# mwaurawakati/hotstuff-digital-signature-benchmarking

Measured on AMD Instinct MI355X. Metric: Ed25519 verifies/sec at batch 2^20 per GPU (bit-exact ed25519-dalek verify_strict flags), higher is better.
Workload: dtype u32; 1 GPU; C4: 2^20 independent (pk, 32-B digest, sig) triples per GPU, inputs resident in HBM; batch_per_gpu=1048576, global_batch=1048576, parallelism=dp1 (contiguous shards, no collective on the data path), kernel_variant=21, streams=3

## Files before the change

### hotstuff-digital-signature-benchmarking_amd/csrc/hsv_kernels.hip

```cpp
#include <hip/hip_runtime.h>

#include <algorithm>
#include <cstdlib>
#include <cstring>
#include <type_traits>
#include <atomic>
#include <mutex>
#include <unordered_map>

#include "hsv_internal.h"
#include "hsv_verify_core.hpp"
#include "hsv_verify_hc.hpp"
#include "hsv_rowpoint.hpp"
#include "hsv_pointpass.hpp"
#include "hsv_msgwave.hpp"

namespace hsv {

#ifdef HSV_PHASE_CLOCKS
constexpr uint32_t kPhaseCap = 1u << 16;
__device__ uint64_t g_phase_clk[kPhaseCap * 8];
#endif

template <int WA>
__global__ void __launch_bounds__(kBlock)
hsv_prep_kernel(const uint8_t *__restrict__ pk, uint64_t pk_stride, const uint8_t *__restrict__ sig,
                uint64_t sig_stride, const uint8_t *__restrict__ msg, uint64_t msg_stride, uint32_t n,
                uint32_t *__restrict__ rec, HcCounters *__restrict__ ctr, uint32_t *__restrict__ fb_list,
                int lat_bits) {
  __builtin_amdgcn_s_setprio(3);
  const uint32_t idx = blockIdx.x * kBlock + threadIdx.x;
  if (idx >= n) return;
  uint32_t pkw[8], sigw[16], msgw[8];
  load_triple(pk, pk_stride, sig, sig_stride, msg, msg_stride, idx, pkw, sigw, msgw);
  if (prep_scalars<WA>(pkw, sigw, msgw, rec + idx, n, lat_bits)) fb_list[atomicAdd(&ctr->fb_count, 1u)] = idx;
}

template <int WA, int WAVES, int CB, bool KREC = false>
__global__ void __launch_bounds__(kBlock, WAVES)
hsv_verify_hp_kernel(const uint8_t *__restrict__ pk, uint64_t pk_stride, const uint8_t *__restrict__ sig,
                     uint64_t sig_stride, const uint8_t *__restrict__ msg, uint64_t msg_stride, uint32_t n,
                     uint8_t *__restrict__ flags_out, uint32_t *__restrict__ strict_bits,
                     uint4 *__restrict__ vt_ws, const uint32_t *__restrict__ comb_b,
                     const uint32_t *__restrict__ rec, HcCounters *__restrict__ ctr,
                     const uint32_t *__restrict__ fb_list, uint32_t *__restrict__ canary, uint32_t nonce,
                     uint32_t inject, uint32_t *__restrict__ fault) {
  constexpr int kEnt = (1 << (WA - 1)) + 1;
  const uint32_t slot = blockIdx.x * kBlock + threadIdx.x;
  GlobalVarTab<kEnt> vt{vt_ws + (uint64_t)slot * vt_lane_uint4<WA>(), inject};
  const uint32_t lane = threadIdx.x & 63u;
  canary[slot] = nonce;
  uint32_t bad = 0;
  const uint32_t nfb = __builtin_amdgcn_readfirstlane(ctr->fb_count);
  const uint32_t fb_end = (nfb + 63u) & ~63u;
  const uint32_t words = (n + 31u) / 32u;
#ifdef HSV_PHASE_CLOCKS
  uint32_t nbw = 0;
#endif
  for (;;) {
    uint32_t base = 0;
    if (lane == 0) base = atomicAdd(&ctr->next, 64u);
    base = __builtin_amdgcn_readfirstlane(__shfl(base, 0));
    if (base >= fb_end + n) break;
    if (inject == kInjectCanary) canary[slot] = ~nonce;
    if (base < fb_end) {
      const uint32_t j = base + lane;
      const bool valid = j < nfb;
      const uint32_t idx = fb_list[valid ? j : base];
      uint32_t pkw[8], sigw[16];
      uint32_t f;
      if constexpr (KREC) {
        const uint4 *p = reinterpret_cast<const uint4 *>(pk + (uint64_t)idx * pk_stride);
        const uint4 *s = reinterpret_cast<const uint4 *>(sig + (uint64_t)idx * sig_stride);
        HSV_UNROLL
        for (int j = 0; j < 2; ++j) {
          const uint4 v = p[j];
          pkw[4 * j] = v.x; pkw[4 * j + 1] = v.y; pkw[4 * j + 2] = v.z; pkw[4 * j + 3] = v.w;
        }
        HSV_UNROLL
        for (int j = 0; j < 4; ++j) {
          const uint4 v = s[j];
          sigw[4 * j] = v.x; sigw[4 * j + 1] = v.y; sigw[4 * j + 2] = v.z; sigw[4 * j + 3] = v.w;
        }
        sc k;
        HSV_UNROLL
        for (int i = 0; i < 8; ++i) k.v[i] = rec[(10ull + (uint64_t)i) * n + idx];
        f = verify_one_full_comb<WA, false, CB>(pkw, sigw, k, comb_b, vt);
      } else {
        uint32_t msgw[8];
        load_triple(pk, pk_stride, sig, sig_stride, msg, msg_stride, idx, pkw, sigw, msgw);
        f = verify_one_full_comb<WA, false, CB>(pkw, sigw, msgw, comb_b, vt);
      }
      bad |= ((f & kFault) ? 1u : 0u) | (canary[slot] != nonce ? 2u : 0u);
      if (valid) {
        if (flags_out) flags_out[idx] = (uint8_t)f;
        if (strict_bits && (f & kStrictOk)) atomicOr(&strict_bits[idx >> 5], 1u << (idx & 31u));
      }
      continue;
    }
    const uint32_t b0 = base - fb_end;
    const uint32_t idx = b0 + lane;
    const bool valid = idx < n;
    const uint32_t li = valid ? idx : n - 1u;
    uint32_t pkw[8], rw[8];
    {
      const uint4 *p = reinterpret_cast<const uint4 *>(pk + (uint64_t)li * pk_stride);
      const uint4 *r = reinterpret_cast<const uint4 *>(sig + (uint64_t)li * sig_stride);
      const uint4 p0 = p[0], p1 = p[1], r0 = r[0], r1 = r[1];
      pkw[0] = p0.x; pkw[1] = p0.y; pkw[2] = p0.z; pkw[3] = p0.w;
      pkw[4] = p1.x; pkw[5] = p1.y; pkw[6] = p1.z; pkw[7] = p1.w;
      rw[0] = r0.x; rw[1] = r0.y; rw[2] = r0.z; rw[3] = r0.w;
      rw[4] = r1.x; rw[5] = r1.y; rw[6] = r1.z; rw[7] = r1.w;
    }
    const uint32_t meta = rec[18ull * n + li];
    const bool own = valid && !(meta & kPrepFallback);
#ifdef HSV_PHASE_CLOCKS
    uint64_t clk[5];
    ++nbw;
    const uint64_t cyc0 = clock64();
    clk[0] = wall_clock64();
    const uint32_t f = verify_one_prepped<WA, CB>(pkw, rw, rec + li, n, meta, comb_b, vt, clk);
    clk[4] = wall_clock64();
    {
      uint64_t v = 1;
      HSV_UNROLL
      for (int j = 0; j < 5; ++j) v = lane == (uint32_t)j ? clk[j] : v;
      v = lane == 5u ? (uint64_t)__builtin_amdgcn_s_getreg((31 << 11) | (0 << 6) | 4) : v;
      v = lane == 6u ? ((uint64_t)blockIdx.x << 8 | nbw) : v;
      v = lane == 7u ? (0x100u | (uint64_t)__builtin_amdgcn_s_getreg((3 << 11) | (0 << 6) | 20) |
                        ((clock64() - cyc0) << 16))
                     : v;
      if (lane < 8u && b0 / 64u < kPhaseCap) g_phase_clk[(uint64_t)(b0 / 64u) * 8u + lane] = v;
    }
#else
    const uint32_t f = verify_one_prepped<WA, CB>(pkw, rw, rec + li, n, meta, comb_b, vt);
#endif
    bad |= ((f & kFault) ? 1u : 0u) | (canary[slot] != nonce ? 2u : 0u);
    const uint32_t fo = KREC && (meta & kPrepVoid) ? 0u : f;
    if (own && flags_out) flags_out[idx] = (uint8_t)fo;
    if (strict_bits) {
      const uint64_t mask = __ballot(own && (fo & kStrictOk));
      const uint32_t w = b0 / 32u + lane;
      const uint32_t part = lane ? (uint32_t)(mask >> 32) : (uint32_t)mask;
      if (lane < 2u && w < words && part) atomicOr(&strict_bits[w], part);
    }
  }
  report_faults(fault, bad);
}



template <int CB>
__device__ __forceinline__ ge_ext comb_add_b_half(ge_ext q, const uint32_t s[8], const uint32_t *tb, uint32_t h) {
  constexpr int NP = 256 / CB, HALF = NP / 2;
  constexpr int ENT = 1 << (CB - 1);
  uint32_t sr[9];
  recode_add<9, CB, NP>(s, 8, sr);
  HSV_UNROLL
  for (int i = 0; i < 4; ++i) sr[i] = h ? sr[i + 4] : sr[i];
  HSV_NOUNROLL
  for (int j = 0; j < HALF; ++j) {
    const uint32_t cb = sr[0] & ((1u << CB) - 1u);
    HSV_UNROLL
    for (int i = 0; i < 3; ++i) sr[i] = (sr[i] >> CB) | (sr[i + 1] << (32 - CB));
    sr[3] >>= CB;
    const CombPosTab tpb{tb + (uint64_t)(j + (int)h * HALF) * ENT * kCombEntryWords};
    q = ge_add_niels<true>(q, select_niels<CB>(tpb, cb));
  }
  return q;
}

__device__ __forceinline__ fe fe_swap_pair(const fe &a) {
  fe r;
  HSV_UNROLL
  for (int i = 0; i < kFeLimbs; ++i) r.v[i] = (uint32_t)__shfl_xor((int)a.v[i], 1, 64);
  return r;
}

template <int WA, class VT>
__device__ __forceinline__ void pair_point_phase(uint32_t p, const uint32_t pk[8], const uint32_t rb[8], VT &vt,
                                                 uint32_t &ok, uint32_t &small) {
  constexpr int TS = 1 << (WA - 1);
  uint32_t pt[8];
  HSV_UNROLL
  for (int i = 0; i < 8; ++i) pt[i] = p ? pk[i] : rb[i];
  fe x, y;
  ok = ge_decompress(pt, x, y);
  small = ok & y_is_small_order(y);
// ... 702 lines not shown

uint32_t next_nonce() {
  static std::atomic<uint32_t> ctr{0x9e3779b9u};
  return (ctr.fetch_add(0x61c88646u) * 2654435761u) | 1u;
}


struct TxPrep {
  const uint8_t *txs;
  const uint64_t *offsets;
  uint64_t tx_size;
  uint8_t *records;
};
struct MsgPrep {
  const uint8_t *msgs;
  const uint64_t *offsets;
  uint64_t msg_len, msg_stride;
};

template <int WA, int WAVES, int CB>
hipError_t launch_hp(const uint8_t *pk, uint64_t pk_stride, const uint8_t *sig, uint64_t sig_stride,
                     const uint8_t *msg, uint64_t msg_stride, uint32_t n, uint8_t *flags_out,
                     uint32_t *strict_bits, const uint32_t *comb_b, uint32_t *fault, hipStream_t stream,
                     const TxPrep *tx = nullptr, void *ws_in = nullptr, size_t ws_cap = 0,
                     size_t *ws_need = nullptr, const MsgPrep *mp = nullptr) {
  const void *kern = mp ? reinterpret_cast<const void *>(hsv::hsv_verify_hp_kernel<WA, WAVES, CB, true>)
                        : reinterpret_cast<const void *>(hsv::hsv_verify_hp_kernel<WA, WAVES, CB>);
  int dev = 0;
  hipError_t e = hipGetDevice(&dev);
  if (e != hipSuccess) return e;
  static std::mutex mu;
  static std::unordered_map<int, std::pair<int, int>> slots_per_dev;
  int bpc = 1, cus = 1;
  {
    std::lock_guard<std::mutex> lk(mu);
    auto it = slots_per_dev.find(2 * dev + (mp ? 1 : 0));
    if (it == slots_per_dev.end()) {
      int b = 0, c = 0;
      e = hipOccupancyMaxActiveBlocksPerMultiprocessor(&b, kern, hsv::kBlock, 0);
      if (e != hipSuccess) return e;
      e = hipDeviceGetAttribute(&c, hipDeviceAttributeMultiprocessorCount, dev);
      if (e != hipSuccess) return e;
      it = slots_per_dev.emplace(2 * dev + (mp ? 1 : 0), std::make_pair(std::max(1, b), std::max(1, c))).first;
    }
    bpc = it->second.first;
    cus = it->second.second;
  }
  const bool fused = tx && WA == 4 && WAVES == HSV_HP_WAVES && CB == 16 && tx_fused_enabled() &&
                     (uint64_t)n * 128u <= 0xffffffffull && hsv_tx_fused_blocks_per_cu(dev) > 0;
  if (fused) bpc = std::min(bpc, hsv_tx_fused_blocks_per_cu(dev));
  const int resident = bpc * (hsvi_resident_started() && cus > 1 ? cus - 1 : cus);
  const uint32_t blocks_needed = (n + hsv::kBlock - 1) / hsv::kBlock;
  const uint32_t grid = std::min<uint32_t>(blocks_needed, (uint32_t)resident);
  const size_t ws_bytes = (size_t)grid * hsv::kBlock * hsv::vt_lane_uint4<WA>() * sizeof(uint4);
  const size_t canary_bytes = ((size_t)grid * hsv::kBlock * sizeof(uint32_t) + 255) & ~(size_t)255;
  const size_t fb_bytes = (size_t)n * sizeof(uint32_t);
  const size_t rec_bytes = (size_t)n * hsv::kPrepWords * sizeof(uint32_t);
  const size_t ready_bytes = fused ? (((size_t)(n + 63u) / 64u) * sizeof(uint32_t) + 255) & ~(size_t)255 : 0;
  const size_t need = ws_bytes + 256 + canary_bytes + fb_bytes + rec_bytes + ready_bytes;
  if (ws_need) {
    *ws_need = need;
    return hipSuccess;
  }
  hsv::Workspace ws(ws_in, ws_cap, need, stream);
  if (ws.status() != hipSuccess) return ws.status();
  uint8_t *ws8 = ws.get();
  uint4 *vt_ws = reinterpret_cast<uint4 *>(ws8);
  hsv::HcCounters *ctr = reinterpret_cast<hsv::HcCounters *>(ws8 + ws_bytes);
  uint32_t *canary = reinterpret_cast<uint32_t *>(ws8 + ws_bytes + 256);
  uint32_t *fb_list = reinterpret_cast<uint32_t *>(ws8 + ws_bytes + 256 + canary_bytes);
  uint32_t *rec = reinterpret_cast<uint32_t *>(ws8 + ws_bytes + 256 + canary_bytes + fb_bytes);
  uint32_t *ready = reinterpret_cast<uint32_t *>(ws8 + ws_bytes + 256 + canary_bytes + fb_bytes + rec_bytes);
  e = hipMemsetAsync(ctr, 0, sizeof(hsv::HcCounters), stream);
  if (e == hipSuccess && strict_bits) e = hipMemsetAsync(strict_bits, 0, (size_t)((n + 31u) / 32u) * 4u, stream);
  if (e == hipSuccess && fused) {
    e = hipMemsetAsync(ready, 0, ready_bytes, stream);
    if (e == hipSuccess)
      e = hsv_launch_tx_fused(grid, tx->txs, tx->offsets, tx->tx_size, n, tx->records, rec, ctr, fb_list, ready,
                              g_lat_bits.load(), flags_out, strict_bits, vt_ws, comb_b, canary, next_nonce(), t_inject,
                              fault, stream);
    return ws.done(e);
  }
  if (e == hipSuccess && tx) {
    static_assert(WA == 4, "hsv_launch_tx_prep writes the WA = 4 prepass record");
    e = hsv_launch_tx_prep(tx->txs, tx->offsets, tx->tx_size, n, tx->records, rec, &ctr->fb_count, fb_list,
                           g_lat_bits.load(), stream);
    pk = tx->records;
    sig = tx->records + 32;
    msg = tx->records + 96;
    pk_stride = sig_stride = msg_stride = 128;
  } else if (e == hipSuccess && mp) {
    static_assert(WA == 4, "hsv_launch_msg_prep writes the WA = 4 prepass record");
    e = hsv_launch_msg_prep(pk, pk_stride, sig, sig_stride, mp->msgs, mp->offsets, mp->msg_len, mp->msg_stride, n,
                            rec, &ctr->fb_count, fb_list, g_lat_bits.load(), stream);
  } else if (e == hipSuccess) {
    hipLaunchKernelGGL((hsv::hsv_prep_kernel<WA>), dim3(blocks_needed), dim3(hsv::kBlock), 0, stream, pk, pk_stride,
                       sig, sig_stride, msg, msg_stride, n, rec, ctr, fb_list, g_lat_bits.load());
    e = hipGetLastError();
  }
  if (e == hipSuccess) {
    if (mp) {
      hipLaunchKernelGGL((hsv::hsv_verify_hp_kernel<WA, WAVES, CB, true>), dim3(grid), dim3(hsv::kBlock), 0, stream,
                         pk, pk_stride, sig, sig_stride, nullptr, 0, n, flags_out, strict_bits, vt_ws, comb_b, rec,
                         ctr, fb_list, canary, next_nonce(), t_inject, fault);
    } else {
      hipLaunchKernelGGL((hsv::hsv_verify_hp_kernel<WA, WAVES, CB>), dim3(grid), dim3(hsv::kBlock), 0, stream, pk,
                         pk_stride, sig, sig_stride, msg, msg_stride, n, flags_out, strict_bits, vt_ws, comb_b, rec,
                         ctr, fb_list, canary, next_nonce(), t_inject, fault);
    }
    e = hipGetLastError();
  }
  return ws.done(e);
}

constexpr uint32_t kPairMax = 1u << 13;
constexpr uint32_t kRowMaxDefault = 3072;

constexpr uint32_t row_max() { return kRowMaxDefault; }

constexpr uint32_t kMsgQuadMax = hsv::kQuadMax;
constexpr uint32_t kMsgJointMax = hsv::kJointMax;
constexpr uint32_t kMsgRowMax = kRowMaxDefault;
enum SmallFormId : int { kFormQuad = 1, kFormJoint = 2, kFormRow = 3, kFormPair = 4 };

template <int WA, int CB, bool MSG = false>
struct SmallForm {
  decltype(&hsv::hsv_verify_quad_kernel<WA, CB, MSG>) kern;
  uint32_t grid, block;
  size_t slots;
  int id;
  explicit SmallForm(uint32_t n, int force = 0) {
    id = force                                        ? force
         : n <= (MSG ? kMsgQuadMax : hsv::kQuadMax)   ? kFormQuad
         : n <= (MSG ? kMsgJointMax : hsv::kJointMax) ? kFormJoint
         : n <= (MSG ? kMsgRowMax : row_max())        ? kFormRow
                                                      : kFormPair;
    if (id == kFormQuad) {
      kern = hsv::hsv_verify_quad_kernel<WA, CB, MSG>;
      grid = n, block = 4 * 64, slots = (size_t)grid * 2u;
    } else if (id == kFormJoint) {
      kern = hsv::hsv_verify_joint_kernel<WA, CB, MSG>;
      grid = (n + hsv::kJointItems - 1) / hsv::kJointItems, block = (hsv::kJointItems + 1) * 64;
      slots = (size_t)grid * hsv::kJointItems;
    } else if (id == kFormRow) {
      kern = hsv::hsv_verify_row_kernel<WA, CB, 1, MSG>;
// ... 238 lines not shown
```

### hotstuff-digital-signature-benchmarking_amd/csrc/hsv_mempool.hip

```cpp
#include <hip/hip_runtime.h>

#include <algorithm>
#include <mutex>
#include <unordered_map>

#define HSV_SHA_BITOP3 1
#include "hsv_internal.h"
#include "hsv_keytab.hpp"
#include "hsv_stage.hpp"
#include "hsv_txhash.hpp"
#include "hsv_verify_hc.hpp"
#include "hsv_pointpass.hpp"
#include "hsv_routed.hpp"

namespace hsv {

constexpr int kTxBlock = 256;

__device__ __forceinline__ bool tx_span(const uint64_t *offsets, uint64_t tx_size, uint32_t i, uint64_t &lo,
                                        uint64_t &hi) {
  if (offsets) {
    lo = offsets[i];
    hi = offsets[i + 1];
  } else {
// ... 40 lines not shown
  const uint64_t q_last = ok ? (start + (hi - lo) - 1) >> 4 : kNoChunk;
  uint64_t h[8];
  sha512_init(h);
  const uint64_t nblocks = tx_num_blocks(mlen);
  uint32_t wave_blocks = (uint32_t)nblocks;
  HSV_UNROLL
  for (int m = 1; m < 64; m <<= 1) wave_blocks = max(wave_blocks, (uint32_t)__shfl_xor((int)wave_blocks, m, 64));
  const uint32_t sh16 = (uint32_t)(start & 15u);
  const bool wave_aligned = __all(sh16 == 0u);
  HSV_NOUNROLL
  for (uint32_t b = 0; b < wave_blocks; ++b) {
    uint32_t raw[4 * kTxQ + 1];
    tx_stage_chunks<kTxQ>(q, stage, lane, (start >> 4) + 8ull * b, q_last, raw);
    const bool wave_full = __all((uint64_t)(b + 1u) * 128u <= mlen);
    if (b < nblocks) {
      uint32_t words[32];
      if (wave_aligned) {
        HSV_UNROLL
        for (int j = 0; j < 32; ++j) words[j] = raw[j];
      } else {
        tx_realign<32>(raw, sh16, words);
      }
      if (wave_full) tx_compress_full_block(h, words);
      else tx_compress_block(h, words, mlen, b, nblocks);
    }
  }
  {
    const uint64_t tail = start + mlen;
    uint32_t raw[4 * 7 + 1];
    tx_stage_chunks<7>(q, stage, lane, tail >> 4, q_last, raw);
    tx_realign<24>(raw, (uint32_t)(tail & 15u), r);
  }
  tx_digest_words(h, r + 24);
  if (!ok) {
    HSV_UNROLL
    for (int j = 0; j < 32; ++j) r[j] = 0u;
  }
  return ok;
}

template <bool PREP, bool CLAMP, class Rec, class Put>
__device__ __forceinline__ void tx_record_lane(const uint8_t *__restrict__ txs, const uint64_t *__restrict__ offsets,
                                               uint64_t tx_size, uint32_t n, uint32_t i_in, uint32_t lane,
                                               uint4 *stage, const Rec &out, uint32_t *__restrict__ prep,
                                               uint32_t *__restrict__ fb_count, uint32_t *__restrict__ fb_list,
                                               int lat_bits) {
  const uint32_t i = CLAMP && i_in >= n ? n - 1u : i_in;
  uint32_t r[32];
  (void)tx_record_words(txs, offsets, tx_size, n, i, lane, stage, r);
  if (CLAMP || i < n) {
    HSV_UNROLL
    for (int j = 0; j < 8; ++j) out.put(i, j, r);
    if constexpr (PREP) {
      const bool fallback = prep_scalars<4, Put>(r, r + 8, r + 24, prep + i, n, lat_bits);
      if (fallback && i == i_in) Put::u32(fb_list + atomicAdd(fb_count, 1u), i);
    }
  }
}

template <bool PREP>
__global__ void __launch_bounds__(kTxBlock) hsv_tx_record_kernel(const uint8_t *__restrict__ txs,
                                                                  const uint64_t *__restrict__ offsets,
                                                                  uint64_t tx_size, uint32_t n,
                                                                  uint4 *__restrict__ rec,
                                                                  uint32_t *__restrict__ prep,
                                                                  uint32_t *__restrict__ fb_count,
                                                                  uint32_t *__restrict__ fb_list, int lat_bits) {
  __shared__ uint4 stage_all[kTxWaves][64 * kTxQ];
  if constexpr (PREP) __builtin_amdgcn_s_setprio(3);
  const uint32_t lane = threadIdx.x & 63u, wv = threadIdx.x >> 6;
  if (blockIdx.x * kTxBlock + wv * 64u >= n) return;
  tx_record_lane<PREP, false, TxRecPlain, PutPlain>(txs, offsets, tx_size, n, blockIdx.x * kTxBlock + threadIdx.x, lane,
                                             stage_all[wv], TxRecPlain{rec}, prep, fb_count, fb_list, lat_bits);
}

constexpr uint64_t kTxFusedWaitTicks = 50000000ull;

__device__ __forceinline__ bool tx_wait_word(uint32_t *w, uint32_t want) {
  const uint64_t t0 = wall_clock64();
  for (;;) {
    const uint32_t v = __builtin_amdgcn_readfirstlane(__hip_atomic_load((gu32 *)w, __ATOMIC_RELAXED, __HIP_MEMORY_SCOPE_AGENT));
    if (v >= want) return true;
    if (wall_clock64() - t0 > kTxFusedWaitTicks) return false;
    __builtin_amdgcn_s_sleep(8);
  }
}

template <int WA, int WAVES, int CB>
__global__ void __launch_bounds__(kBlock, WAVES)
hsv_verify_tx_fused_kernel(const uint8_t *__restrict__ txs, const uint64_t *__restrict__ offsets, uint64_t tx_size,
                           uint32_t n, uint8_t *__restrict__ records,
                           uint32_t *__restrict__ rec, HcCounters *__restrict__ ctr, uint32_t *__restrict__ fb_list,
                           uint32_t *__restrict__ ready, int lat_bits, uint8_t *__restrict__ flags_out,
                           uint32_t *__restrict__ strict_bits, uint4 *__restrict__ vt_ws,
                           const uint32_t *__restrict__ comb_b, uint32_t *__restrict__ canary, uint32_t nonce,
                           uint32_t inject, uint32_t *__restrict__ fault) {
  static_assert(kBlock == kTxBlock, "one staging slot per wave");
  __shared__ uint4 stage_all[kBlock / 64][64 * kTxQ];
  constexpr int kEnt = (1 << (WA - 1)) + 1;
  const uint32_t slot = blockIdx.x * kBlock + threadIdx.x;
  GlobalVarTab<kEnt> vt{vt_ws + (uint64_t)slot * vt_lane_uint4<WA>(), inject};
  const uint32_t lane = threadIdx.x & 63u;
  uint4 *stage = stage_all[threadIdx.x >> 6];
  canary[slot] = nonce;
  uint32_t bad = 0;
  const uint32_t nbatch = (n + 63u) / 64u;
  const __amdgpu_buffer_rsrc_t rec_rsrc = __builtin_amdgcn_make_buffer_rsrc(records, 0, (int)(n * 128u), 0x00020000);
  __builtin_amdgcn_s_setprio(3);
  for (;;) {
    uint32_t rb = 0;
    if (lane == 0) rb = atomicAdd(&ctr->rnext, 1u);
    rb = __builtin_amdgcn_readfirstlane(__shfl(rb, 0));
    if (rb >= nbatch) break;
    tx_record_lane<true, true, TxRecWriteThrough, PutWriteThrough>(txs, offsets, tx_size, n, rb * 64u + lane, lane, stage,
                                                             TxRecWriteThrough{rec_rsrc}, rec, &ctr->fb_count,
                                                             fb_list, lat_bits);
    asm volatile("s_waitcnt vmcnt(0)" ::: "memory");
    if (lane < 2u && !(inject == kInjectNoPublish && rb == 0u))
      __hip_atomic_fetch_add((gu32 *)(lane ? &ctr->rdone : ready + rb), 1u, __ATOMIC_RELAXED, __HIP_MEMORY_SCOPE_AGENT);
  }
  __builtin_amdgcn_s_setprio(0);
  const uint32_t words = (n + 31u) / 32u;
  for (;;) {
    uint32_t base = 0;
    if (lane == 0) base = atomicAdd(&ctr->next, 64u);
    base = __builtin_amdgcn_readfirstlane(__shfl(base, 0));
    if (base >= n) break;
    if (inject == kInjectCanary) canary[slot] = ~nonce;
    if ((bad & 4u) || !tx_wait_word(ready + base / 64u, 1u)) {
      bad |= 5u;
      continue;
    }
    __builtin_amdgcn_fence(__ATOMIC_ACQUIRE, "agent");
    const uint32_t idx = base + lane;
    const bool valid = idx < n;
    const uint32_t li = valid ? idx : n - 1u;
    uint32_t pkw[8], rw[8];
    {
      const uint4 *p = reinterpret_cast<const uint4 *>(records + (uint64_t)li * 128u);
      const uint4 p0 = p[0], p1 = p[1], r0 = p[2], r1 = p[3];
      pkw[0] = p0.x; pkw[1] = p0.y; pkw[2] = p0.z; pkw[3] = p0.w;
      pkw[4] = p1.x; pkw[5] = p1.y; pkw[6] = p1.z; pkw[7] = p1.w;
      rw[0] = r0.x; rw[1] = r0.y; rw[2] = r0.z; rw[3] = r0.w;
      rw[4] = r1.x; rw[5] = r1.y; rw[6] = r1.z; rw[7] = r1.w;
    }
    const uint32_t meta = rec[18ull * n + li];
    const bool own = valid && !(meta & kPrepFallback);
    const uint32_t f = verify_one_prepped<WA, CB>(pkw, rw, rec + li, n, meta, comb_b, vt);
    bad |= ((f & kFault) ? 1u : 0u) | (canary[slot] != nonce ? 2u : 0u);
    if (own && flags_out) flags_out[idx] = (uint8_t)f;
    if (strict_bits) {
      const uint64_t mask = __ballot(own && (f & kStrictOk));
      const uint32_t w = base / 32u + lane;
      const uint32_t part = lane ? (uint32_t)(mask >> 32) : (uint32_t)mask;
      if (lane < 2u && w < words && part) atomicOr(&strict_bits[w], part);
    }
  }
  if (!(bad & 4u) && tx_wait_word(&ctr->rdone, nbatch)) {
    __builtin_amdgcn_fence(__ATOMIC_ACQUIRE, "agent");
    const uint32_t nfb =
        __builtin_amdgcn_readfirstlane(__hip_atomic_load((gu32 *)&ctr->fb_count, __ATOMIC_RELAXED, __HIP_MEMORY_SCOPE_AGENT));
    for (;;) {
      uint32_t base = 0;
      if (lane == 0) base = atomicAdd(&ctr->fb_next, 64u);
      base = __builtin_amdgcn_readfirstlane(__shfl(base, 0));
      if (base >= nfb) break;
      const uint32_t j = base + lane;
      const bool valid = j < nfb;
      const uint32_t idx = fb_list[valid ? j : base];
      uint32_t pkw[8], sigw[16], msgw[8];
      load_triple(records, 128, records + 32, 128, records + 96, 128, idx, pkw, sigw, msgw);
      const uint32_t f = verify_one_full_comb<WA, false, CB>(pkw, sigw, msgw, comb_b, vt);
      bad |= ((f & kFault) ? 1u : 0u) | (canary[slot] != nonce ? 2u : 0u);
      if (valid) {
        if (flags_out) flags_out[idx] = (uint8_t)f;
        if (strict_bits && (f & kStrictOk)) atomicOr(&strict_bits[idx >> 5], 1u << (idx & 31u));
      }
    }
  } else {
    bad |= 1u;
  }
  report_faults(fault, bad & 3u);
}

__global__ void __launch_bounds__(kTxBlock) hsv_tx_mask_kernel(const uint64_t *__restrict__ offsets, uint32_t n,
                                                                uint8_t *flags, uint32_t *strict_bits) {
  const uint32_t i = blockIdx.x * kTxBlock + threadIdx.x;
  if (i >= n) return;
  uint64_t lo, hi;
  if (tx_span(offsets, 0, i, lo, hi)) return;
  if (flags) flags[i] = 0;
  if (strict_bits) atomicAnd(strict_bits + (i >> 5), ~(1u << (i & 31u)));
}

__global__ void __launch_bounds__(kTxBlock)
hsv_ctx_route_kernel(const uint8_t *__restrict__ txs, const uint64_t *__restrict__ offsets, uint64_t tx_size, uint32_t n,
                     uint4 *__restrict__ rec, const uint32_t *__restrict__ keytab, uint32_t keymask, uint64_t seed,
                     const uint8_t *__restrict__ pks, uint32_t nkeys, RoutedCounters *__restrict__ ctr,
                     uint2 *__restrict__ hit_list, uint32_t *__restrict__ miss_list, uint32_t *__restrict__ prep,
                     uint32_t *__restrict__ fb_list, int lat_bits, uint8_t *__restrict__ flags_out) {
  __shared__ uint4 stage_all[kTxWaves][64 * kTxQ];
// ... 269 lines not shown
```

### hotstuff-digital-signature-benchmarking_amd/csrc/hsv_msgs.hip

```cpp
#include <hip/hip_runtime.h>

#define HSV_SHA_BITOP3 1
#include "hsv_internal.h"
#include "hsv_msgwave.hpp"
#include "hsv_verify_hc.hpp"

namespace hsv {

__global__ void __launch_bounds__(kMsgBlock)
hsv_msg_prep_kernel(const uint8_t *__restrict__ pk, uint64_t pk_stride, const uint8_t *__restrict__ sig,
                    uint64_t sig_stride, const uint8_t *__restrict__ msgs, const uint64_t *__restrict__ offsets,
                    uint64_t msg_len, uint64_t msg_stride, uint32_t n, uint32_t *__restrict__ prep,
                    uint32_t *__restrict__ fb_count, uint32_t *__restrict__ fb_list, int lat_bits) {
  __shared__ uint4 stage_all[kMsgWaves][64 * kMsgQ];
  __builtin_amdgcn_s_setprio(3);
  const uint32_t lane = threadIdx.x & 63u, wv = threadIdx.x >> 6;
  if (blockIdx.x * kMsgBlock + wv * 64u >= n) return;
  uint4 *stage = stage_all[wv];
  const uint32_t i_in = blockIdx.x * kMsgBlock + threadIdx.x;
  const uint32_t i = i_in < n ? i_in : n - 1u;
  uint32_t hw[16], s[8];
  const bool ok = msg_hash_lane(pk, pk_stride, sig, sig_stride, msgs, offsets, msg_len, msg_stride, i, lane, stage, hw);
  {
    const uint4 *sigq = reinterpret_cast<const uint4 *>(sig + (uint64_t)i * sig_stride);
    const uint4 s0 = sigq[2], s1 = sigq[3];
    s[0] = s0.x; s[1] = s0.y; s[2] = s0.z; s[3] = s0.w;
    s[4] = s1.x; s[5] = s1.y; s[6] = s1.z; s[7] = s1.w;
  }
  if (i_in < n) {
    const bool fallback = prep_from_hash<4, PutPlain, true>(hw, s, prep + i, n, lat_bits, !ok);
    if (fallback) fb_list[atomicAdd(fb_count, 1u)] = i;
  }
}

}

extern "C" hipError_t hsv_launch_msg_prep(const uint8_t *pk, uint64_t pk_stride, const uint8_t *sig,
                                          uint64_t sig_stride, const uint8_t *msgs, const uint64_t *offsets,
                                          uint64_t msg_len, uint64_t msg_stride, uint32_t n, uint32_t *prep,
                                          uint32_t *fb_count, uint32_t *fb_list, int lat_bits, hipStream_t stream) {
  if (n == 0) return hipSuccess;
  const uint32_t grid = (n + hsv::kMsgBlock - 1) / hsv::kMsgBlock;
  hipLaunchKernelGGL(hsv::hsv_msg_prep_kernel, dim3(grid), dim3(hsv::kMsgBlock), 0, stream, pk, pk_stride, sig,
                     sig_stride, msgs, offsets, msg_len, msg_stride, n, prep, fb_count, fb_list, lat_bits);
  return hipGetLastError();
}
```

### hotstuff-digital-signature-benchmarking_amd/csrc/hsv_pointpass.hpp

```cpp
#pragma once
#include <hip/hip_runtime.h>

#include "hsv_verify_core.hpp"

#ifndef HSV_HP_WAVES
#define HSV_HP_WAVES 3
#endif

namespace hsv {

constexpr int kBlock = 256;


__device__ const uint4 kVtIdentity[8] = {{1u, 0u, 0u, 0u}, {0u, 0u, 0u, 0u}, {1u, 0u, 0u, 0u}, {0u, 0u, 0u, 0u},
                                         {2u, 0u, 0u, 0u}, {0u, 0u, 0u, 0u}, {0u, 0u, 0u, 0u}, {0u, 0u, 0u, 0u}};

template <int ENT>
struct GlobalVarTab {
  static constexpr int kStored = ENT - 1;
  uint4 *base;
  uint32_t inject = kInjectNone;
  __device__ __forceinline__ void put(int t, int m, const uint32_t w[32]) const {
    if (m == 0) return;
    uint4 *e = base + (t * kStored + m - 1) * 8;
    if (__builtin_expect(inject == kInjectZeroTables || (inject == kInjectFlipTables && t == 0), 0)) {
      HSV_UNROLL
      for (int q = 0; q < 8; ++q)
        e[q] = inject == kInjectZeroTables ? make_uint4(0u, 0u, 0u, 0u)
                                           : make_uint4(w[4 * q] ^ (q == 0 ? 1u : 0u), w[4 * q + 1], w[4 * q + 2],
                                                        w[4 * q + 3]);
      return;
    }
    HSV_UNROLL
    for (int q = 0; q < 8; ++q) {
#ifdef HSV_TIMING_STUB_TABLE_STORES
      asm volatile("" ::"v"(w[4 * q]), "v"(w[4 * q + 1]), "v"(w[4 * q + 2]), "v"(w[4 * q + 3]));
#else
      e[q] = make_uint4(w[4 * q], w[4 * q + 1], w[4 * q + 2], w[4 * q + 3]);
#endif
    }
  }
  __device__ __forceinline__ void get(int t, uint32_t m, uint32_t w[32]) const {
    const uint4 *e = m ? base + (t * kStored + (int)m - 1) * 8 : kVtIdentity;
    HSV_UNROLL
    for (int q = 0; q < 8; ++q) {
      const uint4 v = e[q];
      w[4 * q] = v.x; w[4 * q + 1] = v.y; w[4 * q + 2] = v.z; w[4 * q + 3] = v.w;
    }
  }
};

template <int WA>
constexpr int vt_lane_uint4() { return 2 * (1 << (WA - 1)) * 8; }


__device__ __forceinline__ void load_triple(const uint8_t *pk, uint64_t pk_stride, const uint8_t *sig,
                                            uint64_t sig_stride, const uint8_t *msg, uint64_t msg_stride,
                                            uint64_t i, uint32_t pkw[8], uint32_t sigw[16], uint32_t msgw[8]) {
  const uint4 *p = reinterpret_cast<const uint4 *>(pk + i * pk_stride);
  const uint4 *s = reinterpret_cast<const uint4 *>(sig + i * sig_stride);
  const uint4 *m = reinterpret_cast<const uint4 *>(msg + i * msg_stride);
  const uint4 p0 = p[0], p1 = p[1];
  const uint4 s0 = s[0], s1 = s[1], s2 = s[2], s3 = s[3];
  const uint4 m0 = m[0], m1 = m[1];
  pkw[0] = p0.x; pkw[1] = p0.y; pkw[2] = p0.z; pkw[3] = p0.w;
  pkw[4] = p1.x; pkw[5] = p1.y; pkw[6] = p1.z; pkw[7] = p1.w;
  sigw[0] = s0.x; sigw[1] = s0.y; sigw[2] = s0.z; sigw[3] = s0.w;
  sigw[4] = s1.x; sigw[5] = s1.y; sigw[6] = s1.z; sigw[7] = s1.w;
  sigw[8] = s2.x; sigw[9] = s2.y; sigw[10] = s2.z; sigw[11] = s2.w;
  sigw[12] = s3.x; sigw[13] = s3.y; sigw[14] = s3.z; sigw[15] = s3.w;
  msgw[0] = m0.x; msgw[1] = m0.y; msgw[2] = m0.z; msgw[3] = m0.w;
  msgw[4] = m1.x; msgw[5] = m1.y; msgw[6] = m1.z; msgw[7] = m1.w;
}

struct HcCounters {
  uint32_t next;
  uint32_t fb_count;
  uint32_t fb_next;
  uint32_t pad;
  uint32_t rnext;
  uint32_t rdone;
  uint32_t pad2[2];
};

__device__ __forceinline__ void report_faults(uint32_t *fault, uint32_t bad) {
  if (bad & 1u) fault[0] = 1u;
  if (bad & 2u) fault[1] = 1u;
}

}
```

### hotstuff-digital-signature-benchmarking_amd/csrc/hsv_verify_hc.hpp

```cpp
#pragma once
#include "hsv_comb.hpp"
#include "hsv_lattice.hpp"
#include "hsv_verify_core.hpp"

namespace hsv {

template <int CB>
HSV_INL ge_ext comb_add_b(ge_ext q, const uint32_t s[8], const uint32_t *tb) {
  static_assert(CB == 8 || CB == 16, "comb digit width");
#ifdef HSV_TIMING_STUB_COMB
  return q;
#endif
  constexpr int NP = 256 / CB;
  constexpr int ENT = 1 << (CB - 1);
  uint32_t sr[9];
  recode_add<9, CB, NP>(s, 8, sr);
  HSV_NOUNROLL
  for (int j = 0; j < NP; ++j) {
    const uint32_t cb = sr[0] & ((1u << CB) - 1u);
    HSV_UNROLL
    for (int i = 0; i < 8; ++i) sr[i] = (sr[i] >> CB) | (sr[i + 1] << (32 - CB));
    sr[8] >>= CB;
    const CombPosTab tpb{tb + (uint64_t)j * ENT * kCombEntryWords};
    q = ge_add_niels<true>(q, select_niels<CB>(tpb, cb));
// ... 115 lines not shown
  return verify_one_full_comb<WA, PREFETCH, CB>(pk, sig, k, tb, vt);
}

template <int WA>
struct HalfCombWindows {
  static constexpr int NW = (kLatCombBits + 1 + WA) / WA;
  static constexpr int BITS = NW * WA;
  static_assert(BITS <= 160 && BITS >= kLatCombBits + 2, "scalar bound vs loop length");
};

template <int WA, bool PREFETCH = true, int CB = 8, class VT>
HSV_INL uint32_t verify_one_half_comb(const uint32_t pk[8], const uint32_t sig[16], const uint32_t msg[8],
                                      const uint32_t *tb, VT &vt, bool &fallback, int lat_bits = kLatCombBits) {
  using G = HalfCombWindows<WA>;
  constexpr int TS = 1 << (WA - 1);
  const uint32_t s_ok = sc_is_canonical(sig + 8);
  uint32_t h[16];
  sha512_96(sig, pk, msg, h);
  const sc k = sc_reduce512(h);

  uint32_t a_ok, small_a, r_ok, small_r;
  {
    fe x, y;
    r_ok = ge_decompress(sig, x, y);
    small_r = r_ok & y_is_small_order(y);
    vt_build<TS>(vt, 0, fe_carry(fe_neg(x)), y);
  }
  {
    fe x, y;
    a_ok = ge_decompress(pk, x, y);
    small_a = a_ok & y_is_small_order(y);
    vt_build<TS>(vt, 1, fe_carry(fe_neg(x)), y);
  }
  const LatOut lat = lattice_reduce(k, lat_bits);
  fallback = !lat.ok;
  uint32_t d[2][5];
  recode_top5<WA, G::NW>(lat.c1, d[0]);
  recode_top5<WA, G::NW>(lat.c0, d[1]);
  ge_ext q = straus_vt<WA, G::NW, 5, 2, PREFETCH>(d, vt, lat.c0_neg);
  const sc b = sc_mul_small(lat.c1, sig + 8);
  q = comb_add_b<CB>(q, b.v, tb);
  const uint32_t same = ge_is_neutral(q);
  return flags_byte(s_ok, a_ok, r_ok, small_a, small_r, same) | fault_bit(a_ok, r_ok, q);
}

constexpr int kPrepWords = 19;
enum : uint32_t { kPrepSOk = 1u, kPrepC0Neg = 2u, kPrepFallback = 4u };

struct PutPlain {
  static HSV_MEMBER void u32(uint32_t *p, uint32_t v) { *p = v; }
};

constexpr uint32_t kPrepVoid = 8u;
template <int WA, class Put = PutPlain, bool KREC = false>
HSV_INL bool prep_from_hash(const uint32_t h[16], const uint32_t s[8], uint32_t *rec, uint64_t stride,
                            int lat_bits = kLatCombBits, bool skip = false) {
  using G = HalfCombWindows<WA>;
  const uint32_t s_ok = sc_is_canonical(s);
  const sc k = sc_reduce512(h);
  const LatOut lat = lattice_reduce(k, lat_bits);
  uint32_t d[5];
  recode_top5<WA, G::NW>(lat.c1, d);
  HSV_UNROLL
  for (int i = 0; i < 5; ++i) Put::u32(rec + i * stride, d[i]);
  recode_top5<WA, G::NW>(lat.c0, d);
  HSV_UNROLL
  for (int i = 0; i < 5; ++i) Put::u32(rec + (5 + i) * stride, d[i]);
  const sc b = sc_mul_small(lat.c1, s);
  HSV_UNROLL
  for (int i = 0; i < 8; ++i) Put::u32(rec + (10 + i) * stride, KREC && !lat.ok ? k.v[i] : b.v[i]);
  const uint32_t meta = (s_ok ? kPrepSOk : 0u) | (lat.c0_neg ? kPrepC0Neg : 0u) | (lat.ok ? 0u : kPrepFallback);
  Put::u32(rec + 18 * stride, KREC && skip ? kPrepVoid : meta);
  return !lat.ok && !(KREC && skip);
}

template <int WA, class Put = PutPlain>
HSV_INL bool prep_scalars(const uint32_t pk[8], const uint32_t sig[16], const uint32_t msg[8], uint32_t *rec,
                          uint64_t stride, int lat_bits = kLatCombBits) {
  uint32_t h[16];
  sha512_96(sig, pk, msg, h);
  return prep_from_hash<WA, Put>(h, sig + 8, rec, stride, lat_bits);
}

#ifdef HSV_PHASE_CLOCKS
#define HSV_CLK(j)                       \
  do {                                   \
    if (clk) clk[j] = wall_clock64();    \
  } while (0)
#else
#define HSV_CLK(j) \
  do {             \
  } while (0)
#endif

template <int WA, int CB, class VT>
HSV_INL uint32_t verify_one_prepped(const uint32_t pk[8], const uint32_t rb[8], const uint32_t *rec,
                                    uint64_t stride, const uint32_t meta, const uint32_t *tb, VT &vt,
                                    uint64_t *clk = nullptr) {
  using G = HalfCombWindows<WA>;
  constexpr int TS = 1 << (WA - 1);
  uint32_t a_ok, small_a, r_ok, small_r;
  {
    fe xr, yr, xa, ya;
    ge_decompress2(rb, pk, xr, yr, xa, ya, r_ok, a_ok);
    small_r = r_ok & y_is_small_order(yr);
    small_a = a_ok & y_is_small_order(ya);
    HSV_CLK(1);
    vt_build<TS>(vt, 0, fe_carry(fe_neg(xr)), yr);
    vt_build<TS>(vt, 1, fe_carry(fe_neg(xa)), ya);
    HSV_CLK(2);
  }
  uint32_t d[2][5];
  HSV_UNROLL
  for (int i = 0; i < 5; ++i) {
    d[0][i] = rec[i * stride];
    d[1][i] = rec[(5 + i) * stride];
  }
  ge_ext q = straus_vt<WA, G::NW, 5, 2, false>(d, vt, (meta & kPrepC0Neg) ? 1u : 0u);
  HSV_CLK(3);
  uint32_t b[8];
  HSV_UNROLL
  for (int i = 0; i < 8; ++i) b[i] = rec[(10 + i) * stride];
  q = comb_add_b<CB>(q, b, tb);
  const uint32_t same = ge_is_neutral(q);
  return flags_byte(meta & kPrepSOk, a_ok, r_ok, small_a, small_r, same) | fault_bit(a_ok, r_ok, q);
}

}
```

Before: 118.5 million verif/s.

## Replace two separate window-4 Straus tables with a joint 2-bit point-pass table

Replaces the per-point window-4 variable-base tables and Straus loop for R and A with a single joint table of signed combinations 5i+j (i,j in -2..2), indexed by 2-bit signed digits of both half scalars. Each column now does one cached-point add plus two doublings instead of one add per point per window. The prep kernels recode scalars into 2-bit digits to match. This trades fewer table builds and fewer additions for more columns and a different global-memory table layout (12 lines per lane).

```diff
diff --git a/hotstuff-digital-signature-benchmarking_amd/csrc/hsv_kernels.hip b/hotstuff-digital-signature-benchmarking_amd/csrc/hsv_kernels.hip
--- a/hotstuff-digital-signature-benchmarking_amd/csrc/hsv_kernels.hip
+++ b/hotstuff-digital-signature-benchmarking_amd/csrc/hsv_kernels.hip
@@ -33,7 +33,8 @@
   if (idx >= n) return;
   uint32_t pkw[8], sigw[16], msgw[8];
   load_triple(pk, pk_stride, sig, sig_stride, msg, msg_stride, idx, pkw, sigw, msgw);
-  if (prep_scalars<WA>(pkw, sigw, msgw, rec + idx, n, lat_bits)) fb_list[atomicAdd(&ctr->fb_count, 1u)] = idx;
+  if (prep_scalars<WA, PutPlain, pointpass_digit_bits<WA>()>(pkw, sigw, msgw, rec + idx, n, lat_bits))
+    fb_list[atomicAdd(&ctr->fb_count, 1u)] = idx;
 }
 
 template <int WA, int WAVES, int CB, bool KREC = false>
@@ -45,9 +46,9 @@
                      const uint32_t *__restrict__ rec, HcCounters *__restrict__ ctr,
                      const uint32_t *__restrict__ fb_list, uint32_t *__restrict__ canary, uint32_t nonce,
                      uint32_t inject, uint32_t *__restrict__ fault) {
-  constexpr int kEnt = (1 << (WA - 1)) + 1;
+  constexpr bool JOINT = joint_pointpass<WA>();
   const uint32_t slot = blockIdx.x * kBlock + threadIdx.x;
-  GlobalVarTab<kEnt> vt{vt_ws + (uint64_t)slot * vt_lane_uint4<WA>(), inject};
+  PointPassTab<WA> vt{vt_ws + (uint64_t)slot * pointpass_lane_uint4<WA>(), inject};
   const uint32_t lane = threadIdx.x & 63u;
   canary[slot] = nonce;
   uint32_t bad = 0;
@@ -119,7 +120,7 @@
     ++nbw;
     const uint64_t cyc0 = clock64();
     clk[0] = wall_clock64();
-    const uint32_t f = verify_one_prepped<WA, CB>(pkw, rw, rec + li, n, meta, comb_b, vt, clk);
+    const uint32_t f = verify_one_prepped<WA, CB, JOINT>(pkw, rw, rec + li, n, meta, comb_b, vt, clk);
     clk[4] = wall_clock64();
     {
       uint64_t v = 1;
@@ -133,7 +134,7 @@
       if (lane < 8u && b0 / 64u < kPhaseCap) g_phase_clk[(uint64_t)(b0 / 64u) * 8u + lane] = v;
     }
 #else
-    const uint32_t f = verify_one_prepped<WA, CB>(pkw, rw, rec + li, n, meta, comb_b, vt);
+    const uint32_t f = verify_one_prepped<WA, CB, JOINT>(pkw, rw, rec + li, n, meta, comb_b, vt);
 #endif
     bad |= ((f & kFault) ? 1u : 0u) | (canary[slot] != nonce ? 2u : 0u);
     const uint32_t fo = KREC && (meta & kPrepVoid) ? 0u : f;
@@ -942,7 +943,7 @@
   const int resident = bpc * (hsvi_resident_started() && cus > 1 ? cus - 1 : cus);
   const uint32_t blocks_needed = (n + hsv::kBlock - 1) / hsv::kBlock;
   const uint32_t grid = std::min<uint32_t>(blocks_needed, (uint32_t)resident);
-  const size_t ws_bytes = (size_t)grid * hsv::kBlock * hsv::vt_lane_uint4<WA>() * sizeof(uint4);
+  const size_t ws_bytes = (size_t)grid * hsv::kBlock * hsv::pointpass_lane_uint4<WA>() * sizeof(uint4);
   const size_t canary_bytes = ((size_t)grid * hsv::kBlock * sizeof(uint32_t) + 255) & ~(size_t)255;
   const size_t fb_bytes = (size_t)n * sizeof(uint32_t);
   const size_t rec_bytes = (size_t)n * hsv::kPrepWords * sizeof(uint32_t);
@@ -972,7 +973,7 @@
     return ws.done(e);
   }
   if (e == hipSuccess && tx) {
-    static_assert(WA == 4, "hsv_launch_tx_prep writes the WA = 4 prepass record");
+    static_assert(WA == 4, "hsv_launch_tx_prep writes the WA = 4 point pass's prepass record");
     e = hsv_launch_tx_prep(tx->txs, tx->offsets, tx->tx_size, n, tx->records, rec, &ctr->fb_count, fb_list,
                            g_lat_bits.load(), stream);
     pk = tx->records;
@@ -980,7 +981,7 @@
     msg = tx->records + 96;
     pk_stride = sig_stride = msg_stride = 128;
   } else if (e == hipSuccess && mp) {
-    static_assert(WA == 4, "hsv_launch_msg_prep writes the WA = 4 prepass record");
+    static_assert(WA == 4, "hsv_launch_msg_prep writes the WA = 4 point pass's prepass record");
     e = hsv_launch_msg_prep(pk, pk_stride, sig, sig_stride, mp->msgs, mp->offsets, mp->msg_len, mp->msg_stride, n,
                             rec, &ctr->fb_count, fb_list, g_lat_bits.load(), stream);
   } else if (e == hipSuccess) {
diff --git a/hotstuff-digital-signature-benchmarking_amd/csrc/hsv_mempool.hip b/hotstuff-digital-signature-benchmarking_amd/csrc/hsv_mempool.hip
--- a/hotstuff-digital-signature-benchmarking_amd/csrc/hsv_mempool.hip
+++ b/hotstuff-digital-signature-benchmarking_amd/csrc/hsv_mempool.hip
@@ -116,7 +116,7 @@
     HSV_UNROLL
     for (int j = 0; j < 8; ++j) out.put(i, j, r);
     if constexpr (PREP) {
-      const bool fallback = prep_scalars<4, Put>(r, r + 8, r + 24, prep + i, n, lat_bits);
+      const bool fallback = prep_scalars<4, Put, pointpass_digit_bits<4>()>(r, r + 8, r + 24, prep + i, n, lat_bits);
       if (fallback && i == i_in) Put::u32(fb_list + atomicAdd(fb_count, 1u), i);
     }
   }
@@ -161,9 +161,8 @@
                            uint32_t inject, uint32_t *__restrict__ fault) {
   static_assert(kBlock == kTxBlock, "one staging slot per wave");
   __shared__ uint4 stage_all[kBlock / 64][64 * kTxQ];
-  constexpr int kEnt = (1 << (WA - 1)) + 1;
   const uint32_t slot = blockIdx.x * kBlock + threadIdx.x;
-  GlobalVarTab<kEnt> vt{vt_ws + (uint64_t)slot * vt_lane_uint4<WA>(), inject};
+  PointPassTab<WA> vt{vt_ws + (uint64_t)slot * pointpass_lane_uint4<WA>(), inject};
   const uint32_t lane = threadIdx.x & 63u;
   uint4 *stage = stage_all[threadIdx.x >> 6];
   canary[slot] = nonce;
@@ -210,7 +209,7 @@
     }
     const uint32_t meta = rec[18ull * n + li];
     const bool own = valid && !(meta & kPrepFallback);
-    const uint32_t f = verify_one_prepped<WA, CB>(pkw, rw, rec + li, n, meta, comb_b, vt);
+    const uint32_t f = verify_one_prepped<WA, CB, joint_pointpass<WA>()>(pkw, rw, rec + li, n, meta, comb_b, vt);
     bad |= ((f & kFault) ? 1u : 0u) | (canary[slot] != nonce ? 2u : 0u);
     if (own && flags_out) flags_out[idx] = (uint8_t)f;
     if (strict_bits) {
diff --git a/hotstuff-digital-signature-benchmarking_amd/csrc/hsv_msgs.hip b/hotstuff-digital-signature-benchmarking_amd/csrc/hsv_msgs.hip
--- a/hotstuff-digital-signature-benchmarking_amd/csrc/hsv_msgs.hip
+++ b/hotstuff-digital-signature-benchmarking_amd/csrc/hsv_msgs.hip
@@ -28,7 +28,7 @@
     s[4] = s1.x; s[5] = s1.y; s[6] = s1.z; s[7] = s1.w;
   }
   if (i_in < n) {
-    const bool fallback = prep_from_hash<4, PutPlain, true>(hw, s, prep + i, n, lat_bits, !ok);
+    const bool fallback = prep_from_hash<4, PutPlain, true, pointpass_digit_bits<4>()>(hw, s, prep + i, n, lat_bits, !ok);
     if (fallback) fb_list[atomicAdd(fb_count, 1u)] = i;
   }
 }
diff --git a/hotstuff-digital-signature-benchmarking_amd/csrc/hsv_pointpass.hpp b/hotstuff-digital-signature-benchmarking_amd/csrc/hsv_pointpass.hpp
--- a/hotstuff-digital-signature-benchmarking_amd/csrc/hsv_pointpass.hpp
+++ b/hotstuff-digital-signature-benchmarking_amd/csrc/hsv_pointpass.hpp
@@ -1,7 +1,10 @@
 #pragma once
 #include <hip/hip_runtime.h>
 
+#include <type_traits>
+
 #include "hsv_verify_core.hpp"
+#include "hsv_verify_hc.hpp"
 
 #ifndef HSV_HP_WAVES
 #define HSV_HP_WAVES 3
@@ -53,6 +56,51 @@
 template <int WA>
 constexpr int vt_lane_uint4() { return 2 * (1 << (WA - 1)) * 8; }
 
+struct GlobalJointTab {
+  uint4 *base;
+  uint32_t inject = kInjectNone;
+  __device__ __forceinline__ void put(int t, int m, const uint32_t w[32]) const {
+    GlobalVarTab<9>{base, inject}.put(t, m, w);
+  }
+  __device__ __forceinline__ void get(int t, uint32_t m, uint32_t w[32]) const {
+    GlobalVarTab<9>{base, inject}.get(t, m, w);
+  }
+  __device__ __forceinline__ void put_line(uint32_t l, const uint32_t w[32]) const {
+    uint4 *e = base + (l - 1u) * 8u;
+    if (__builtin_expect(inject == kInjectZeroTables || (inject == kInjectFlipTables && l >= kJointFirstLineOfR), 0)) {
+      HSV_UNROLL
+      for (int q = 0; q < 8; ++q)
+        e[q] = inject == kInjectZeroTables ? make_uint4(0u, 0u, 0u, 0u)
+                                           : make_uint4(w[4 * q] ^ (q == 0 ? 1u : 0u), w[4 * q + 1], w[4 * q + 2],
+                                                        w[4 * q + 3]);
+      return;
+    }
+    HSV_UNROLL
+    for (int q = 0; q < 8; ++q) {
+#ifdef HSV_TIMING_STUB_TABLE_STORES
+      asm volatile("" ::"v"(w[4 * q]), "v"(w[4 * q + 1]), "v"(w[4 * q + 2]), "v"(w[4 * q + 3]));
+#else
+      e[q] = make_uint4(w[4 * q], w[4 * q + 1], w[4 * q + 2], w[4 * q + 3]);
+#endif
+    }
+  }
+  __device__ __forceinline__ void get_line(uint32_t l, uint32_t w[32]) const {
+    const uint4 *e = l ? base + (l - 1u) * 8u : kVtIdentity;
+    HSV_UNROLL
+    for (int q = 0; q < 8; ++q) {
+      const uint4 v = e[q];
+      w[4 * q] = v.x; w[4 * q + 1] = v.y; w[4 * q + 2] = v.z; w[4 * q + 3] = v.w;
+    }
+  }
+};
+constexpr int kJointLaneUint4 = kJointLines * 8;
+static_assert(kJointLines >= 8, "the fallback path's 8-line table shares the slot");
+
+template <int WA>
+using PointPassTab = std::conditional_t<joint_pointpass<WA>(), GlobalJointTab, GlobalVarTab<(1 << (WA - 1)) + 1>>;
+template <int WA>
+constexpr int pointpass_lane_uint4() { return joint_pointpass<WA>() ? kJointLaneUint4 : vt_lane_uint4<WA>(); }
+
 
 __device__ __forceinline__ void load_triple(const uint8_t *pk, uint64_t pk_stride, const uint8_t *sig,
                                             uint64_t sig_stride, const uint8_t *msg, uint64_t msg_stride,
diff --git a/hotstuff-digital-signature-benchmarking_amd/csrc/hsv_verify_hc.hpp b/hotstuff-digital-signature-benchmarking_amd/csrc/hsv_verify_hc.hpp
--- a/hotstuff-digital-signature-benchmarking_amd/csrc/hsv_verify_hc.hpp
+++ b/hotstuff-digital-signature-benchmarking_amd/csrc/hsv_verify_hc.hpp
@@ -191,18 +191,20 @@
 };
 
 constexpr uint32_t kPrepVoid = 8u;
-template <int WA, class Put = PutPlain, bool KREC = false>
+static_assert(kLatCombBits + 2 <= HalfCombWindows<2>::BITS && HalfCombWindows<2>::NW == 70,
+              "2-bit columns: c < 2^138 plus the recoding constant (0.667 * 2^140) must stay below 2^140");
+template <int WA, class Put = PutPlain, bool KREC = false, int DW = WA>
 HSV_INL bool prep_from_hash(const uint32_t h[16], const uint32_t s[8], uint32_t *rec, uint64_t stride,
                             int lat_bits = kLatCombBits, bool skip = false) {
-  using G = HalfCombWindows<WA>;
+  using G = HalfCombWindows<DW>;
   const uint32_t s_ok = sc_is_canonical(s);
   const sc k = sc_reduce512(h);
   const LatOut lat = lattice_reduce(k, lat_bits);
   uint32_t d[5];
-  recode_top5<WA, G::NW>(lat.c1, d);
+  recode_top5<DW, G::NW>(lat.c1, d);
   HSV_UNROLL
   for (int i = 0; i < 5; ++i) Put::u32(rec + i * stride, d[i]);
-  recode_top5<WA, G::NW>(lat.c0, d);
+  recode_top5<DW, G::NW>(lat.c0, d);
   HSV_UNROLL
   for (int i = 0; i < 5; ++i) Put::u32(rec + (5 + i) * stride, d[i]);
   const sc b = sc_mul_small(lat.c1, s);
@@ -213,12 +215,12 @@
   return !lat.ok && !(KREC && skip);
 }
 
-template <int WA, class Put = PutPlain>
+template <int WA, class Put = PutPlain, int DW = WA>
 HSV_INL bool prep_scalars(const uint32_t pk[8], const uint32_t sig[16], const uint32_t msg[8], uint32_t *rec,
                           uint64_t stride, int lat_bits = kLatCombBits) {
   uint32_t h[16];
   sha512_96(sig, pk, msg, h);
-  return prep_from_hash<WA, Put>(h, sig + 8, rec, stride, lat_bits);
+  return prep_from_hash<WA, Put, false, DW>(h, sig + 8, rec, stride, lat_bits);
 }
 
 #ifdef HSV_PHASE_CLOCKS
@@ -232,11 +234,113 @@
   } while (0)
 #endif
 
-template <int WA, int CB, class VT>
+constexpr int kJointLines = 12;
+constexpr uint32_t kJointFirstLineOfR = 3;
+
+HSV_INL uint32_t joint_line(int i, int j, uint32_t &neg) {
+  const int s = 5 * i + j;
+  neg = s < 0;
+  return (uint32_t)(s < 0 ? -s : s);
+}
+
+HSV_INL uint32_t joint_column(uint32_t ci, uint32_t cj, uint32_t flip, uint32_t &neg) {
+  const int j = (int)cj - 2;
+  return joint_line((int)ci - 2, flip ? -j : j, neg);
+}
+
+template <class VT>
+HSV_INL void jt_put(VT &vt, uint32_t line, const ge_ext &p) {
+  uint32_t w[32];
+  cached_pack(ge_to_cached(p), w);
+  vt.put_line(line, w);
+}
+
+template <class VT>
+HSV_INL void jt_pair(VT &vt, const ge_ext &p, const ge_cached &q, uint32_t ls, uint32_t ld) {
+  const fe a = fe_sub(p.Y, p.X), b = fe_add(p.Y, p.X);
+  fe A, B, A2, B2, C, D;
+  fe_mul2(p.T, q.T2d, p.Z, q.Z2, C, D);
+  fe_mul2(a, q.YmX, b, q.YpX, A, B);
+  fe_mul2(a, q.YpX, b, q.YmX, A2, B2);
+  const fe F = fe_sub(D, C), G = fe_add(D, C);
+  jt_put(vt, ls, ge_finish_rt(fe_sub(B, A), F, G, fe_add(B, A), true));
+  jt_put(vt, ld, ge_finish_rt(fe_sub(B2, A2), G, F, fe_add(B2, A2), true));
+}
+
+template <class VT>
+HSV_INL void jt_build(VT &vt, const fe &xp, const fe &yp, const fe &xq, const fe &yq) {
+#ifdef HSV_TIMING_STUB_TABLES
+  return;
+#endif
+  ge_ext p, q;
+  p.X = xp;
+  p.Y = yp;
+  p.Z = fe_small(1);
+  q.X = xq;
+  q.Y = yq;
+  q.Z = fe_small(1);
+  fe_mul2(xp, yp, xq, yq, p.T, q.T);
+  uint32_t neg;
+  jt_put(vt, joint_line(0, 1, neg), q);
+  jt_put(vt, joint_line(0, 2, neg), ge_dbl_rt(q, true));
+  HSV_NOUNROLL
+  for (int i = 1; i <= 2; ++i) {
+    if (i == 2) p = ge_dbl_rt(p, true);
+    jt_put(vt, joint_line(i, 0, neg), p);
+    HSV_NOUNROLL
+    for (int j = 1; j <= 2; ++j) {
+      uint32_t w[32];
+      vt.get_line(joint_line(0, j, neg), w);
+      jt_pair(vt, p, cached_unpack(w), joint_line(i, j, neg), joint_line(i, -j, neg));
+    }
+  }
+}
+
+template <int NW, class VT>
+HSV_INL ge_ext straus_joint(uint32_t d[2][5], VT &vt, uint32_t flip) {
+  ge_ext q = ge_identity();
+#ifdef HSV_TIMING_STUB_STRAUS
+  return q;
+#endif
+  int top = NW - 1;
+  HSV_NOUNROLL
+  while (top > 0) {
+    const uint32_t nz = ((d[0][4] >> 30) ^ 2u) | ((d[1][4] >> 30) ^ 2u);
+    if (wave_any(nz)) break;
+    limbs_shl<5>(d[0], 2);
+    limbs_shl<5>(d[1], 2);
+    --top;
+  }
+  HSV_NOUNROLL
+  for (int c = top; c >= 0; --c) {
+    uint32_t neg;
+    const uint32_t line = joint_column(d[0][4] >> 30, d[1][4] >> 30, flip, neg);
+    limbs_shl<5>(d[0], 2);
+    limbs_shl<5>(d[1], 2);
+    if (c != top) {
+      HSV_NOUNROLL
+      for (int j = 0; j < 2; ++j) q = ge_dbl_rt(q, j == 1);
+    }
+    uint32_t cur[32];
+    vt.get_line(line, cur);
+    q = ge_add_cached_rt(q, ge_cached_cneg(cached_unpack(cur), neg), c == 0);
+  }
+  return q;
+}
+
+#ifndef HSV_JOINT_POINTPASS
+#define HSV_JOINT_POINTPASS 1
+#endif
+template <int WA>
+constexpr bool joint_pointpass() { return HSV_JOINT_POINTPASS && WA == 4; }
+template <int WA>
+constexpr int pointpass_digit_bits() { return joint_pointpass<WA>() ? 2 : WA; }
+
+template <int WA, int CB, bool JOINT = false, class VT>
 HSV_INL uint32_t verify_one_prepped(const uint32_t pk[8], const uint32_t rb[8], const uint32_t *rec,
                                     uint64_t stride, const uint32_t meta, const uint32_t *tb, VT &vt,
                                     uint64_t *clk = nullptr) {
-  using G = HalfCombWindows<WA>;
+  using G = HalfCombWindows<JOINT ? 2 : WA>;
   constexpr int TS = 1 << (WA - 1);
   uint32_t a_ok, small_a, r_ok, small_r;
   {
@@ -245,8 +349,12 @@
     small_r = r_ok & y_is_small_order(yr);
     small_a = a_ok & y_is_small_order(ya);
     HSV_CLK(1);
-    vt_build<TS>(vt, 0, fe_carry(fe_neg(xr)), yr);
-    vt_build<TS>(vt, 1, fe_carry(fe_neg(xa)), ya);
+    if constexpr (JOINT) {
+      jt_build(vt, fe_carry(fe_neg(xr)), yr, fe_carry(fe_neg(xa)), ya);
+    } else {
+      vt_build<TS>(vt, 0, fe_carry(fe_neg(xr)), yr);
+      vt_build<TS>(vt, 1, fe_carry(fe_neg(xa)), ya);
+    }
     HSV_CLK(2);
   }
   uint32_t d[2][5];
@@ -255,7 +363,10 @@
     d[0][i] = rec[i * stride];
     d[1][i] = rec[(5 + i) * stride];
   }
-  ge_ext q = straus_vt<WA, G::NW, 5, 2, false>(d, vt, (meta & kPrepC0Neg) ? 1u : 0u);
+  const uint32_t c0_neg = (meta & kPrepC0Neg) ? 1u : 0u;
+  ge_ext q;
+  if constexpr (JOINT) q = straus_joint<G::NW>(d, vt, c0_neg);
+  else q = straus_vt<WA, G::NW, 5, 2, false>(d, vt, c0_neg);
   HSV_CLK(3);
   uint32_t b[8];
   HSV_UNROLL
```

New measurement: 121.0 million verif/s (median of 6 runs). 1.02x the previous value.
